# Skylarking/MARL

Hardware: AMD Instinct MI355X
Metric: env_steps_per_sec (higher is better)
Workload: dtype f32 (bf16x6 split products, fp32 accumulate)

## Files before the change

### marl_amd/csrc/qmix_fused.hip

```cpp
#include "x6.h"
#include "../../include/marl_hip.h"

namespace {

constexpr int E = 32;
constexpr int KCQ = 8;
constexpr int SS = 128 + 4;
constexpr int NAG = 5;
constexpr int PP = 136;

struct QmixArgs {
  const float *W[4], *Bv[4];
  const float *wb2, *bb2;
  ConcatSrc s;
  const float* q;
  const float* g;
  float* q_tot;
  float* dq;
  float* ws;
  const float *lr, *lterm, *lpadded, *lq_tgt;
  float gamma;
  long rows;
  int N, S, C;
};

__host__ __device__ inline long qmix_slab_floats(int C, int S) { return (long)C * (S + 1) + (E + 1) + 2; }

template <int CTRL>
__device__ __forceinline__ float dpp(float v) {
  return __builtin_bit_cast(float, __builtin_amdgcn_update_dpp(0, __builtin_bit_cast(int, v), CTRL, 0xf, 0xf, true));
}
constexpr int DPP_XOR1 = 0xB1, DPP_XOR2 = 0x4E;
constexpr int DPP_HALF_MIRROR = 0x141, DPP_MIRROR = 0x140;
constexpr int DPP_ROR4 = 0x124, DPP_ROR8 = 0x128;
template <int EW>
__device__ __forceinline__ float group_sum(float v) {
  if (EW == 4) v += dpp<DPP_ROR4>(v);
  v += dpp<DPP_ROR8>(v);
  return v;
}
template <int EW>
__device__ __forceinline__ float e_sum(float v) {
  v += dpp<DPP_XOR1>(v);
  v += dpp<DPP_XOR2>(v);
  if (EW == 8) v += dpp<DPP_HALF_MIRROR>(v);
  return v;
}
__device__ __forceinline__ float row_sum(float v) {
  v += dpp<DPP_XOR1>(v);
  v += dpp<DPP_XOR2>(v);
  v += dpp<DPP_HALF_MIRROR>(v);
  v += dpp<DPP_MIRROR>(v);
  return v;
}
__device__ __forceinline__ float sign_clamp(float x, float lo) { return __builtin_amdgcn_fmed3f(x * 0x1p126f, lo, 1.0f); }

template <bool BWD, int NW, bool LOSS = false, bool X6 = false>
__global__ __launch_bounds__(64 * NW, 2) void qmix_fused_kernel(QmixArgs a) {
  static_assert(!LOSS || BWD, "the loss is folded into the backward kernel");
  static_assert(!X6 || NW == 8, "the split variant runs eight waves (two column tiles per wave: 96 registers of pre-split weights)");
  constexpr int QNT = 64 * NW, EW = 32 / NW, GPT = 16 / EW, TPW = 8 / GPT, LT = TPW - 1;
  constexpr int SRAW = X6 ? 2 * 3 * 16 * PP * 2 : 2 * 16 * SS * 4;
  __shared__ __attribute__((aligned(16))) char Sraw[SRAW];
  float (*Ss)[16 * SS] = reinterpret_cast<float (*)[16 * SS]>(Sraw);
  short* const Sp = reinterpret_cast<short*>(Sraw);
  constexpr int PLN = 16 * PP, PBUF = 3 * PLN;
  constexpr int KR = (X6 && BWD) ? (LOSS ? 2 : 3) : 4;
  constexpr int KL = 4 - KR;
  __shared__ __attribute__((aligned(16))) i32x4 WL[KL ? NW * TPW * KL * 3 * 64 : 1];
  __shared__ __attribute__((aligned(16))) float Qt2[2][8][16];
  __shared__ __attribute__((aligned(16))) float QT[NW][16];
  __shared__ __attribute__((aligned(16))) float DQP[NW][NAG][16];
  __shared__ __attribute__((aligned(16))) float Gs2[2][16];
  __shared__ __attribute__((aligned(16))) float Ls2[2][4][16];
  const int tid = threadIdx.x, lane = tid & 63, wave = tid >> 6;
  const int q4 = lane >> 4, m = lane & 15;
  const int el = m & (EW - 1), gl = m / EW, e = EW * wave + el;
  const int N = a.N, S = a.S, C = a.C, NE = N * E;
  const bool ones = S < 128;

  f32x4 wq[X6 ? 1 : TPW][X6 ? 1 : KCQ];
  F3 wq6[X6 ? TPW : 1][X6 ? KR : 1];
  float bias[TPW];
  int grp[TPW];
#pragma unroll
  for (int c = 0; c < TPW; ++c) {
    const int g = GPT * c + gl;
    grp[c] = g;
    const float *Wp = nullptr, *Bp = nullptr;
    if (g < NAG) { if (g < N) { Wp = a.W[0] + (long)(g * E + e) * S; Bp = a.Bv[0] + g * E + e; } }
    else { Wp = a.W[g - NAG + 1] + (long)e * S; Bp = a.Bv[g - NAG + 1] + e; }
    bias[c] = Bp ? *Bp : 0.f;
    if (X6) {
#pragma unroll
      for (int kc = 0; kc < 4; ++kc) {
        float v[8];
#pragma unroll
        for (int jj = 0; jj < 8; ++jj) {
          const int kk = 32 * kc + 8 * q4 + jj;
          v[jj] = (Wp && kk < S) ? Wp[kk] : 0.f;
        }
        const F3 f = split8((f32x4){v[0], v[1], v[2], v[3]}, (f32x4){v[4], v[5], v[6], v[7]});
        if (kc < KR) wq6[c][kc < KR ? kc : 0] = f;
        else { i32x4* wl = WL + (((wave * TPW + c) * (KL ? KL : 1) + (kc - KR)) * 3) * 64 + lane; wl[0] = f.h; wl[64] = f.m; wl[128] = f.l; }
      }
    } else {
#pragma unroll
      for (int kc = 0; kc < KCQ; ++kc)
#pragma unroll
        for (int i = 0; i < 4; ++i) {
          const int kk = 16 * kc + 4 * q4 + i;
          wq[c][kc][i] = (Wp && kk < S) ? Wp[kk] : 0.f;
        }
    }
  }
  const bool is6 = grp[LT] == 6, is7 = grp[LT] == 7;
  const float wb2e = a.wb2[e];
  const float cw = is7 ? wb2e : 0.f;
  const float bb2 = a.bb2[0];
  constexpr int MT = NAG / GPT;
  const unsigned absmask = grp[MT] < NAG ? 0x7fffffffu : 0xffffffffu;
  float lo_c[TPW];
#pragma unroll
  for (int c = 0; c < TPW; ++c) lo_c[c] = grp[c] == NAG ? 1.f : (grp[c] == 7 ? 0.f : -1.f);

  f32x4 accW[BWD ? TPW : 1][BWD ? KCQ : 1];
  float sbW[TPW];
#pragma unroll
  for (int c = 0; c < TPW; ++c) sbW[c] = 0.f;
  float acc_wb2 = 0.f, acc_bb2 = 0.f;
  float acc_ln = 0.f, acc_lm = 0.f;
  if (BWD) {
#pragma unroll
    for (int c = 0; c < TPW; ++c)
#pragma unroll
      for (int kc = 0; kc < KCQ; ++kc) accW[c][kc] = (f32x4){0.f, 0.f, 0.f, 0.f};
  }
  if (tid < 2 * 8 * 16) {
    const int r8 = (tid >> 4) & 7;
    (&Qt2[0][0][0])[tid] = r8 == NAG ? 1.f : 0.f;
  }

  const int tiles = (int)((a.rows + 15) / 16);
  constexpr int NPF = 512 / QNT;
  f32x4 pf[NPF];
  int pe0 = 0, pe1 = 0, pw0 = 0, pw1 = 0;
  const int fr = tid >> 5, fc4 = (tid & 31) * 4;
  const bool ones_lane = BWD && ones && fc4 == (S & ~3);
  const int ones_j = S & 3;
  const int nrows = (int)a.rows;
  const unsigned last_row = (unsigned)(nrows - 1);
  const unsigned rpe = (unsigned)a.s.rpe0;
  const int roff = rpe ? (int)a.s.off0 : 0;
  const FastDiv fd = a.s.fd0;
  const int* emap = a.s.emap0;
  const float* sp0 = a.s.p0 + (fc4 < S ? fc4 : 0);
  const long ld = a.s.ld0, blk = (long)a.s.bs0 * a.s.ld0;
  auto map_one = [&](int tile, int i, int& pe, int& pw) {
    unsigned row = (unsigned)tile * 16u + (unsigned)(fr + (QNT / 32) * i);
    row = row < last_row ? row : last_row;
    const unsigned ep = rpe ? fastdiv(row, fd) : 0u;
    pw = (int)(row - ep * rpe) + roff;
    pe = (int)ep;
    if (emap) pe = emap[ep];
  };
  auto map_issue = [&](int tile) {
    map_one(tile, 0, pe0, pw0);
    if (NPF > 1) map_one(tile, 1, pe1, pw1);
  };
  auto fetch_one = [&](int pe, int pw) {
    f32x4 v = *reinterpret_cast<const f32x4*>(sp0 + ((long)pe * blk + (long)pw * ld));
    if (BWD) {
#pragma unroll
      for (int j = 0; j < 4; ++j) v[j] = (ones_lane && j == ones_j) ? 1.f : v[j];
    }
    return v;
  };
  auto fetch = [&](int) {
    pf[0] = fetch_one(pe0, pw0);
    if (NPF > 1) pf[NPF - 1] = fetch_one(pe1, pw1);
  };
  auto stash = [&](int buf) {
#pragma unroll
    for (int i = 0; i < NPF; ++i) {
      if (X6) {
        const F3h f = split4(pf[i]);
        short* p = Sp + buf * PBUF + (fr + (QNT / 32) * i) * PP + fc4;
        *reinterpret_cast<i32x2*>(p) = f.h;
        *reinterpret_cast<i32x2*>(p + PLN) = f.m;
        *reinterpret_cast<i32x2*>(p + 2 * PLN) = f.l;
      } else *reinterpret_cast<f32x4*>(&Ss[buf][(fr + (QNT / 32) * i) * SS + fc4]) = pf[i];
    }
  };
  float pq = 0.f, pg = 0.f, pl[4] = {0.f, 0.f, 0.f, 0.f};
  const int qr = tid / N, qn = tid - qr * N;
  auto fetch_qg = [&](int tile) {
    pq = 0.f; pg = 0.f;
    if (tid < 16 * N) {
      const int row = tile * 16 + qr;
      if (row < nrows) pq = a.q[(unsigned)(row * N + qn)];
    }
    if (BWD && tid >= 192 && tid < 208) {
      const int row = tile * 16 + (tid - 192);
      if (LOSS) {
        pl[0] = pl[1] = pl[3] = 0.f; pl[2] = 1.f;
        if (row < nrows) { pl[0] = a.lr[row]; pl[1] = a.lterm[row]; pl[2] = a.lpadded[row]; pl[3] = a.lq_tgt[row]; }
      } else if (row < nrows) pg = a.g[row];
    }
  };
  auto flush_dq = [&](int prow0) {
    if (tid < 16 * N) {
      float v = 0.f;
#pragma unroll
      for (int w = 0; w < NW; ++w) v += DQP[w][qn][qr];
      if (prow0 + qr < nrows) a.dq[(unsigned)((prow0 + qr) * N + qn)] = v;
    }
  };
  int tile = blockIdx.x;
  if (tile < tiles) {
    map_issue(tile); fetch(tile); fetch_qg(tile);
    if (tile + (int)gridDim.x < tiles) map_issue(tile + gridDim.x);
    stash(0);
  }
  int buf = 0;
  int prow0 = -1;
  ST_DECL(8);
  __syncthreads();
  for (; tile < tiles; tile += gridDim.x, buf ^= 1) {
    const int row0 = tile * 16;
    if (tid < 16 * N) Qt2[buf][qn][qr] = pq;
    if (BWD && tid >= 192 && tid < 208) {
      if (LOSS) {
#pragma unroll
        for (int k = 0; k < 4; ++k) Ls2[buf][k][tid - 192] = pl[k];
      } else Gs2[buf][tid - 192] = pg;
    }
    const int nt = tile + gridDim.x;
    if (nt < tiles) {
      fetch(nt); fetch_qg(nt);
      if (nt + (int)gridDim.x < tiles) map_issue(nt + gridDim.x);
    }
    ST_MARK(0);
    WG_BARRIER();
    ST_MARK(1);
    if (BWD && prow0 >= 0) flush_dq(prow0);
    f32x4 acc[TPW];
#pragma unroll
    for (int c = 0; c < TPW; ++c) acc[c] = (f32x4){bias[c], bias[c], bias[c], bias[c]};
    if (X6) {
      f32x4 accb[TPW];
#pragma unroll
      for (int c = 0; c < TPW; ++c) accb[c] = (f32x4){0.f, 0.f, 0.f, 0.f};
      const short* sp = Sp + buf * PBUF + m * PP + 8 * q4;
#pragma unroll
      for (int kc = 0; kc < 4; ++kc) {
        F3 xa;
        xa.h = *reinterpret_cast<const i32x4*>(sp + 32 * kc);
        xa.m = *reinterpret_cast<const i32x4*>(sp + PLN + 32 * kc);
        xa.l = *reinterpret_cast<const i32x4*>(sp + 2 * PLN + 32 * kc);
        F3 wk[TPW];
#pragma unroll
        for (int c = 0; c < TPW; ++c) {
          if (kc < KR) wk[c] = wq6[c][kc < KR ? kc : 0];
          else { const i32x4* wl = WL + (((wave * TPW + c) * (KL ? KL : 1) + (kc - KR)) * 3) * 64 + lane; wk[c].h = wl[0]; wk[c].m = wl[64]; wk[c].l = wl[128]; }
        }
#define OP(p_, q_) _Pragma("unroll") for (int c = 0; c < TPW; ++c) { if (kc & 1) accb[c] = mm(xa.p_, wk[c].q_, accb[c]); else acc[c] = mm(xa.p_, wk[c].q_, acc[c]); }
        OP(m, m) OP(h, l) OP(l, h) OP(h, m) OP(m, h) OP(h, h)
#undef OP
      }
#pragma unroll
      for (int c = 0; c < TPW; ++c) acc[c] += accb[c];
    } else {
      const float* sr = &Ss[buf][m * SS + 4 * q4];
#pragma unroll
      for (int kc = 0; kc < KCQ; ++kc) {
        const f32x4 a4 = *reinterpret_cast<const f32x4*>(sr + 16 * kc);
#pragma unroll
        for (int i = 0; i < 4; ++i)
#pragma unroll
          for (int c = 0; c < TPW; ++c) acc[c] = mfma16(a4[i], wq[c][kc][i], acc[c]);
      }
    }
    ST_MARK(2);
    __builtin_amdgcn_sched_barrier(0);
    f32x4 qv[TPW];
    f32x4 p = {0.f, 0.f, 0.f, 0.f};
#pragma unroll
    for (int c = 0; c <= MT; ++c) {
      qv[c] = *reinterpret_cast<const f32x4*>(&Qt2[buf][grp[c]][4 * q4]);
#pragma unroll
      for (int i = 0; i < 4; ++i) {
        const float av = acc[c][i];
        const float x = c < MT ? fabsf(av) : __builtin_bit_cast(float, __builtin_bit_cast(unsigned, av) & absmask);
        p[i] = c == 0 ? x * qv[c][i] : fmaf(x, qv[c][i], p[i]);
      }
    }
    f32x4 ex, hid, t4;
#pragma unroll
    for (int i = 0; i < 4; ++i) {
      p[i] = group_sum<EW>(p[i]);
      ex[i] = __expf(p[i]);
      hid[i] = p[i] > 0.f ? p[i] : ex[i] - 1.f;
      const float z = is6 ? fabsf(acc[LT][i]) : fmaxf(acc[LT][i], 0.f);
      t4[i] = row_sum(z * (is6 ? hid[i] : cw));
    }
    if (m == 0) *reinterpret_cast<f32x4*>(&QT[wave][4 * q4]) = t4;
    ST_MARK(3);
    WG_BARRIER();
    ST_MARK(4);
    if (!BWD) {
      if (tid < 16) {
        float tot = 0.f;
#pragma unroll
        for (int w = 0; w < NW; ++w) tot += QT[w][tid];
        if (row0 + tid < nrows) a.q_tot[row0 + tid] = tot + bb2;
      }
      ST_MARK(5);
    } else {
      f32x4 qt = *reinterpret_cast<const f32x4*>(&QT[0][4 * q4]);
#pragma unroll
      for (int w = 1; w < NW; ++w) qt += *reinterpret_cast<const f32x4*>(&QT[w][4 * q4]);
      f32x4 gr;
      if (LOSS) {
        const f32x4 lr = *reinterpret_cast<const f32x4*>(&Ls2[buf][0][4 * q4]);
        const f32x4 lt = *reinterpret_cast<const f32x4*>(&Ls2[buf][1][4 * q4]);
        const f32x4 lp = *reinterpret_cast<const f32x4*>(&Ls2[buf][2][4 * q4]);
        const f32x4 lq = *reinterpret_cast<const f32x4*>(&Ls2[buf][3][4 * q4]);
#pragma unroll
        for (int i = 0; i < 4; ++i) {
          qt[i] += bb2;
          const float mask = 1.f - lp[i];
          const float target = lr[i] + a.gamma * lq[i] * (1.f - lt[i]);
          const float mtd = mask * (target - qt[i]);
          gr[i] = -2.f * mask * mtd;
          acc_ln += mtd * mtd; acc_lm += mask;
        }
        if (a.q_tot && wave == 0 && m == 0) {
          if (row0 + 16 <= nrows) *reinterpret_cast<f32x4*>(&a.q_tot[row0 + 4 * q4]) = qt;
          else {
#pragma unroll
            for (int i = 0; i < 4; ++i) if (row0 + 4 * q4 + i < nrows) a.q_tot[row0 + 4 * q4 + i] = qt[i];
          }
        }
      } else gr = *reinterpret_cast<const f32x4*>(&Gs2[buf][4 * q4]);
      f32x4 dpre, dhy[TPW];
#pragma unroll
      for (int i = 0; i < 4; ++i) {
        const float w2 = group_sum<EW>(is6 ? fabsf(acc[LT][i]) : 0.f);
        dpre[i] = gr[i] * w2 * (p[i] > 0.f ? 1.f : ex[i]);
        acc_wb2 += gr[i] * fmaxf(acc[LT][i], 0.f);
        acc_bb2 += gr[i];
      }
#pragma unroll
      for (int c = 0; c < TPW; ++c) {
        const bool lo_all = GPT * c + GPT - 1 <= NAG, hi_all = GPT * c > NAG;
#pragma unroll
        for (int i = 0; i < 4; ++i) {
          float x, y;
          if (lo_all) { x = qv[c][i]; y = dpre[i]; }
          else if (hi_all) { x = gr[i]; y = is6 ? hid[i] : wb2e; }
          else {
            const bool lo = grp[c] <= NAG;
            x = lo ? qv[c][i] : gr[i];
            y = lo ? dpre[i] : (is6 ? hid[i] : wb2e);
          }
          dhy[c][i] = (x * y) * sign_clamp(acc[c][i], lo_c[c]);
        }
        if (!ones) sbW[c] += dhy[c][0] + dhy[c][1] + dhy[c][2] + dhy[c][3];
        if (GPT * c < NAG) {
          f32x4 d4;
#pragma unroll
          for (int i = 0; i < 4; ++i) d4[i] = e_sum<EW>(fabsf(acc[c][i]) * dpre[i]);
          if (el == 0 && grp[c] < N) *reinterpret_cast<f32x4*>(&DQP[wave][grp[c]][4 * q4]) = d4;
        }
      }
      ST_MARK(5);
      __builtin_amdgcn_sched_barrier(0);
      if (X6) {
        typedef __attribute__((address_space(3))) s16x4 lds_s16x4;
        F3h dA[TPW];
#pragma unroll
        for (int c = 0; c < TPW; ++c) dA[c] = split4(dhy[c]);
        const short* tb = Sp + buf * PBUF + (4 * q4 + (m >> 2)) * PP + 4 * (m & 3);
#pragma unroll
        for (int kc = 0; kc < KCQ; ++kc) {
          F3h sb;
          sb.h = __builtin_bit_cast(i32x2, __builtin_amdgcn_ds_read_tr16_b64_v4i16((lds_s16x4*)(tb + 16 * kc)));
          sb.m = __builtin_bit_cast(i32x2, __builtin_amdgcn_ds_read_tr16_b64_v4i16((lds_s16x4*)(tb + PLN + 16 * kc)));
          sb.l = __builtin_bit_cast(i32x2, __builtin_amdgcn_ds_read_tr16_b64_v4i16((lds_s16x4*)(tb + 2 * PLN + 16 * kc)));
#define OP(p_, q_) _Pragma("unroll") for (int c = 0; c < TPW; ++c) accW[c][kc] = mmh(dA[c].p_, sb.q_, accW[c][kc]);
          OP(m, m) OP(h, l) OP(l, h) OP(h, m) OP(m, h) OP(h, h)
#undef OP
        }
      } else {
        const float* sd = &Ss[buf][(4 * q4) * SS + m];
#pragma unroll
        for (int kc = 0; kc < KCQ; ++kc) {
          f32x4 sD;
#pragma unroll
          for (int i = 0; i < 4; ++i) sD[i] = sd[i * SS + 16 * kc];
#pragma unroll
          for (int i = 0; i < 4; ++i)
#pragma unroll
            for (int c = 0; c < TPW; ++c) accW[c][kc] = mfma16(dhy[c][i], sD[i], accW[c][kc]);
        }
      }
      prow0 = row0;
    }
    ST_MARK(6);
    if (nt < tiles) stash(buf ^ 1);
    ST_MARK(7);
  }
  ST_DUMP_AT(8, BWD ? 8 : 0);
  if (BWD) {
    __syncthreads();
    if (prow0 >= 0) flush_dq(prow0);
    float* slab = a.ws + (long)blockIdx.x * qmix_slab_floats(C, S);
    const int Sx = S + 1;
#pragma unroll
    for (int c = 0; c < TPW; ++c) {
#pragma unroll
      for (int i = 0; i < 4; ++i) {
        const int cc = 4 * q4 + i, g = GPT * c + cc / EW, ee = EW * wave + (cc & (EW - 1));
        if (g < NAG && g >= N) continue;
        const int col = g < NAG ? g * E + ee : NE + (g - NAG) * E + ee;
#pragma unroll
        for (int kc = 0; kc < KCQ; ++kc) {
          const int k = 16 * kc + m;
          if (k < S || (ones && k == S)) slab[(long)col * Sx + k] = accW[c][kc][i];
        }
      }
      if (!ones) {
        float sb = sbW[c];
        sb += __shfl_xor(sb, 16, 64); sb += __shfl_xor(sb, 32, 64);
        const int g = grp[c];
        if (q4 == 0 && !(g < NAG && g >= N)) slab[(long)(g < NAG ? g * E + e : NE + (g - NAG) * E + e) * Sx + S] = sb;
      }
    }
    float v = acc_wb2;
    v += __shfl_xor(v, 16, 64); v += __shfl_xor(v, 32, 64);
    if (is7 && q4 == 0) slab[(long)C * Sx + e] = v;
    float b = acc_bb2, ln = acc_ln, lm = acc_lm;
    b += __shfl_xor(b, 16, 64); b += __shfl_xor(b, 32, 64);
    ln += __shfl_xor(ln, 16, 64); ln += __shfl_xor(ln, 32, 64);
    lm += __shfl_xor(lm, 16, 64); lm += __shfl_xor(lm, 32, 64);
    if (tid == 0) {
      slab[(long)C * Sx + E] = b;
      slab[(long)C * Sx + E + 1] = LOSS ? ln : 0.f;
      slab[(long)C * Sx + E + 2] = LOSS ? lm : 0.f;
    }
  }
}

struct QmixRedArgs {
  const float* ws; int nwg; int N, S, C;
  float *dW[4], *dB[4], *dwb2, *dbb2;
  float* loss2;
};

constexpr int RSG = 16;

__global__ __launch_bounds__(64 * RSG) void qmix_fused_reduce_kernel(QmixRedArgs a) {
  __shared__ float part[RSG][64];
  const long slab = qmix_slab_floats(a.C, a.S);
  const int el = threadIdx.x & 63, sg = threadIdx.x >> 6;
  const long e = (long)blockIdx.x * 64 + el;
  float s = 0.f;
  if (e < slab) s = slab_sum(a.ws + e, slab, sg, RSG, a.nwg);
  part[sg][el] = s;
  __syncthreads();
  if (sg != 0 || e >= slab) return;
  s = 0.f;
#pragma unroll
  for (int g = 0; g < RSG; ++g) s += part[g][el];
  const int Sx = a.S + 1, NE = a.N * E;
  if (e < (long)a.C * Sx) {
    const int col = (int)(e / Sx), k = (int)(e - (long)col * Sx);
    int seg, sc;
    if (col < NE) { seg = 0; sc = col; }
    else if (col < NE + E) { seg = 1; sc = col - NE; }
    else if (col < NE + 2 * E) { seg = 2; sc = col - NE - E; }
    else { seg = 3; sc = col - NE - 2 * E; }
    if (k < a.S) a.dW[seg][(long)sc * a.S + k] += s;
    else a.dB[seg][sc] += s;
  } else {
    const long tpos = e - (long)a.C * Sx;
    if (tpos < E) a.dwb2[tpos] += s;
    else if (tpos == E) a.dbb2[0] += s;
    else if (a.loss2) a.loss2[tpos - E - 1] += s;
  }
}

}
ST_DEFINE_SETTER(marl_debug_stamps_qmix)
namespace {

inline bool supported(int N, int S, int Eq) { return Eq == E && N >= 1 && N <= NAG && S <= 128 && S >= 1; }

inline ConcatSrc state_src(const marl_src_t* s) {
  ConcatSrc c;
  c.p0 = s->p0; c.ld0 = s->ld0; c.k0 = s->k0; c.p1 = nullptr; c.ld1 = 0; c.k1 = 0;
  c.idx = nullptr; c.nhot = 0; c.hot_w = 0; c.nid = 0; c.m0 = nullptr; c.ldm0 = 0;
  c.rpe0 = s->rpe0; c.bs0 = s->bs0; c.off0 = s->off0; c.rpei = 0; c.bsi = 0; c.offi = 0;
  c.fd0 = make_fastdiv((unsigned)(s->rpe0 > 0 ? s->rpe0 : 1));
  c.fdi = make_fastdiv(1); c.fdn = make_fastdiv(1);
  c.emap0 = s->emap0;
  return c;
}

inline int fill(QmixArgs& a, const marl_qmix_weights_t* w, const marl_src_t* s, const float* q, long rows, int N, int S) {
  a.W[0] = w->w1; a.Bv[0] = w->w1_b; a.W[1] = w->b1; a.Bv[1] = w->b1_b; a.W[2] = w->w2; a.Bv[2] = w->w2_b;
  a.W[3] = w->h; a.Bv[3] = w->h_b; a.wb2 = w->b2_w; a.bb2 = w->b2_b;
  a.s = state_src(s);
  if (a.s.k0 != S || s->k1 || s->nhot || s->nid || s->m0 || (a.s.ld0 % 4) || ((uintptr_t)a.s.p0 & 15)) return 1;
  a.q = q; a.rows = rows; a.N = N; a.S = S; a.C = N * E + 3 * E;
  return 0;
}

inline unsigned grid_for(long rows, int per_cu = 1) {
  long tiles = (rows + 15) / 16;
  return (unsigned)(tiles < 256 * per_cu ? tiles : 256 * per_cu);
}

}

extern "C" int marl_qmix_fused_supported(int N, int S, int Eq) { return supported(N, S, Eq) ? 1 : 0; }

extern "C" size_t marl_qmix_fused_workspace(long rows, int N, int S) {
  return (size_t)grid_for(rows) * qmix_slab_floats(N * E + 3 * E, S) * sizeof(float);
}

static int qmix_fwd_impl(const marl_qmix_weights_t* w, const marl_src_t* s, const float* q, float* q_tot,
                         long rows, int N, int S, int Eq, bool x6, void* stream) {
  if (rows <= 0) return 0;
  if (!supported(N, S, Eq)) return (int)hipErrorInvalidValue;
  QmixArgs a;
  if (fill(a, w, s, q, rows, N, S)) return (int)hipErrorInvalidValue;
  a.g = nullptr; a.q_tot = q_tot; a.dq = nullptr; a.ws = nullptr;
  a.lr = a.lterm = a.lpadded = a.lq_tgt = nullptr; a.gamma = 0.f;
  if (x6) hipLaunchKernelGGL((qmix_fused_kernel<false, 8, false, true>), dim3(grid_for(rows, 1)), dim3(512), 0, (hipStream_t)stream, a);
  else hipLaunchKernelGGL((qmix_fused_kernel<false, 4>), dim3(grid_for(rows, 2)), dim3(256), 0, (hipStream_t)stream, a);
  MARL_CHECK_LAUNCH();
  return 0;
}
extern "C" int marl_qmix_fused_fwd(const marl_qmix_weights_t* w, const marl_src_t* s, const float* q, float* q_tot,
                                   long rows, int N, int S, int Eq, void* stream) {
  return qmix_fwd_impl(w, s, q, q_tot, rows, N, S, Eq, false, stream);
}
extern "C" int marl_qmix_fused_fwd_x6(const marl_qmix_weights_t* w, const marl_src_t* s, const float* q, float* q_tot,
                                      long rows, int N, int S, int Eq, void* stream) {
  return qmix_fwd_impl(w, s, q, q_tot, rows, N, S, Eq, true, stream);
}

static int qmix_bwd_launch(QmixArgs& a, const marl_qmix_weights_t* grads, float* loss2, float* ws, long rows, int N, int S,
                           bool loss, bool x6, hipStream_t st) {
  const unsigned nwg = grid_for(rows);
  if (x6) {
    if (loss) hipLaunchKernelGGL((qmix_fused_kernel<true, 8, true, true>), dim3(nwg), dim3(512), 0, st, a);
    else hipLaunchKernelGGL((qmix_fused_kernel<true, 8, false, true>), dim3(nwg), dim3(512), 0, st, a);
  } else if (loss) hipLaunchKernelGGL((qmix_fused_kernel<true, 8, true>), dim3(nwg), dim3(512), 0, st, a);
  else hipLaunchKernelGGL((qmix_fused_kernel<true, 8, false>), dim3(nwg), dim3(512), 0, st, a);
  MARL_CHECK_LAUNCH();
  QmixRedArgs r;
  r.ws = ws; r.nwg = (int)nwg; r.N = N; r.S = S; r.C = a.C; r.loss2 = loss2;
  r.dW[0] = const_cast<float*>(grads->w1); r.dB[0] = const_cast<float*>(grads->w1_b);
  r.dW[1] = const_cast<float*>(grads->b1); r.dB[1] = const_cast<float*>(grads->b1_b);
  r.dW[2] = const_cast<float*>(grads->w2); r.dB[2] = const_cast<float*>(grads->w2_b);
  r.dW[3] = const_cast<float*>(grads->h); r.dB[3] = const_cast<float*>(grads->h_b);
  r.dwb2 = const_cast<float*>(grads->b2_w); r.dbb2 = const_cast<float*>(grads->b2_b);
  const long slab = qmix_slab_floats(a.C, S);
  hipLaunchKernelGGL(qmix_fused_reduce_kernel, dim3((unsigned)((slab + 63) / 64)), dim3(64 * RSG), 0, st, r);
  MARL_CHECK_LAUNCH();
  return 0;
}

static int qmix_bwd_impl(const marl_qmix_weights_t* w, const marl_src_t* s, const float* q, const float* dq_tot, float* dq,
                         const marl_qmix_weights_t* grads, float* ws, size_t ws_bytes, long rows, int N, int S, int Eq, bool x6,
                         void* stream) {
  if (rows <= 0) return 0;
  if (!supported(N, S, Eq)) return (int)hipErrorInvalidValue;
  if (ws_bytes < marl_qmix_fused_workspace(rows, N, S)) return (int)hipErrorInvalidValue;
  QmixArgs a;
  if (fill(a, w, s, q, rows, N, S)) return (int)hipErrorInvalidValue;
  a.g = dq_tot; a.q_tot = nullptr; a.dq = dq; a.ws = ws;
  a.lr = a.lterm = a.lpadded = a.lq_tgt = nullptr; a.gamma = 0.f;
  return qmix_bwd_launch(a, grads, nullptr, ws, rows, N, S, false, x6, (hipStream_t)stream);
}
extern "C" int marl_qmix_fused_bwd(const marl_qmix_weights_t* w, const marl_src_t* s, const float* q,
                                   const float* dq_tot, float* dq, const marl_qmix_weights_t* grads, float* ws,
                                   size_t ws_bytes, long rows, int N, int S, int Eq, void* stream) {
  return qmix_bwd_impl(w, s, q, dq_tot, dq, grads, ws, ws_bytes, rows, N, S, Eq, false, stream);
}
extern "C" int marl_qmix_fused_bwd_x6(const marl_qmix_weights_t* w, const marl_src_t* s, const float* q,
                                      const float* dq_tot, float* dq, const marl_qmix_weights_t* grads, float* ws,
                                      size_t ws_bytes, long rows, int N, int S, int Eq, void* stream) {
  return qmix_bwd_impl(w, s, q, dq_tot, dq, grads, ws, ws_bytes, rows, N, S, Eq, true, stream);
}

static int qmix_loss_bwd_impl(const marl_qmix_weights_t* w, const marl_src_t* s, const float* q,
                              const float* q_tot_tgt, const float* r, const float* term, const float* padded,
                              float gamma, float* q_tot, float* dq, const marl_qmix_weights_t* grads,
                              float* loss2, float* ws, size_t ws_bytes, long rows, int N, int S, int Eq, bool x6,
                              void* stream) {
  if (rows <= 0) return 0;
  if (!supported(N, S, Eq) || !q_tot_tgt || !r || !term || !padded || !loss2) return (int)hipErrorInvalidValue;
  if (reinterpret_cast<uintptr_t>(q_tot) & 15) return (int)hipErrorInvalidValue;
  if (ws_bytes < marl_qmix_fused_workspace(rows, N, S)) return (int)hipErrorInvalidValue;
  QmixArgs a;
  if (fill(a, w, s, q, rows, N, S)) return (int)hipErrorInvalidValue;
  a.g = nullptr; a.q_tot = q_tot; a.dq = dq; a.ws = ws;
  a.lr = r; a.lterm = term; a.lpadded = padded; a.lq_tgt = q_tot_tgt; a.gamma = gamma;
  return qmix_bwd_launch(a, grads, loss2, ws, rows, N, S, true, x6, (hipStream_t)stream);
}
extern "C" int marl_qmix_fused_loss_bwd(const marl_qmix_weights_t* w, const marl_src_t* s, const float* q,
                                        const float* q_tot_tgt, const float* r, const float* term, const float* padded,
                                        float gamma, float* q_tot, float* dq, const marl_qmix_weights_t* grads,
                                        float* loss2, float* ws, size_t ws_bytes, long rows, int N, int S, int Eq,
                                        void* stream) {
  return qmix_loss_bwd_impl(w, s, q, q_tot_tgt, r, term, padded, gamma, q_tot, dq, grads, loss2, ws, ws_bytes, rows, N, S, Eq, false, stream);
}
extern "C" int marl_qmix_fused_loss_bwd_x6(const marl_qmix_weights_t* w, const marl_src_t* s, const float* q,
                                           const float* q_tot_tgt, const float* r, const float* term, const float* padded,
                                           float gamma, float* q_tot, float* dq, const marl_qmix_weights_t* grads,
                                           float* loss2, float* ws, size_t ws_bytes, long rows, int N, int S, int Eq,
                                           void* stream) {
  return qmix_loss_bwd_impl(w, s, q, q_tot_tgt, r, term, padded, gamma, q_tot, dq, grads, loss2, ws, ws_bytes, rows, N, S, Eq, true, stream);
}
```

Measured before the change: 66.50 million.

## Process two row tiles per iteration in the split-precision QMIX kernel

Adds a paired-tile mode for the X6 (bf16x6) path. Each loop iteration now stages, computes the hypernetwork products for, and back-propagates two 16-row tiles. Split weights held in registers or LDS are reused across both tiles, and the number of workgroup barriers per row is halved. To free registers, the backward path keeps fewer pre-split weight chunks in registers, loads biases from LDS, recomputes hid, and re-derives lane indices to lower register pressure. The prefetch and the second tile's elementwise backward are scheduled to overlap with the weight-gradient MFMAs. In exchange it uses more LDS, adds code complexity, and may increase register spills.

```diff
diff --git a/marl_amd/csrc/qmix_fused.hip b/marl_amd/csrc/qmix_fused.hip
--- a/marl_amd/csrc/qmix_fused.hip
+++ b/marl_amd/csrc/qmix_fused.hip
@@ -1,5 +1,18 @@
 #include "x6.h"
 #include "../../include/marl_hip.h"
+
+#ifndef QMIX_PAIR
+#define QMIX_PAIR 3
+#endif
+#ifndef QMIX_PAIR_PF
+#define QMIX_PAIR_PF 1
+#endif
+#ifndef QMIX_PAIR_REINDEX
+#define QMIX_PAIR_REINDEX 1
+#endif
+#ifndef QMIX_PAIR_LATE_B
+#define QMIX_PAIR_LATE_B 1
+#endif
 
 namespace {
 
@@ -55,27 +68,37 @@
 }
 __device__ __forceinline__ float sign_clamp(float x, float lo) { return __builtin_amdgcn_fmed3f(x * 0x1p126f, lo, 1.0f); }
 
+template <int V> struct IC { static constexpr int v = V; };
+template <int TPW>
+struct QTile { f32x4 acc[TPW], qv[TPW], p, ex, hid; };
+
 template <bool BWD, int NW, bool LOSS = false, bool X6 = false>
 __global__ __launch_bounds__(64 * NW, 2) void qmix_fused_kernel(QmixArgs a) {
   static_assert(!LOSS || BWD, "the loss is folded into the backward kernel");
   static_assert(!X6 || NW == 8, "the split variant runs eight waves (two column tiles per wave: 96 registers of pre-split weights)");
   constexpr int QNT = 64 * NW, EW = 32 / NW, GPT = 16 / EW, TPW = 8 / GPT, LT = TPW - 1;
-  constexpr int SRAW = X6 ? 2 * 3 * 16 * PP * 2 : 2 * 16 * SS * 4;
+  constexpr bool PAIR = X6 && ((QMIX_PAIR >> (BWD ? (LOSS ? 2 : 1) : 0)) & 1);
+  constexpr int NSL = PAIR ? 4 : 2, NQT = PAIR ? 2 : 1;
+  constexpr bool EARLY_PUT = PAIR && BWD;
+  constexpr int SRAW = X6 ? NSL * 3 * 16 * PP * 2 : 2 * 16 * SS * 4;
   __shared__ __attribute__((aligned(16))) char Sraw[SRAW];
   float (*Ss)[16 * SS] = reinterpret_cast<float (*)[16 * SS]>(Sraw);
   short* const Sp = reinterpret_cast<short*>(Sraw);
   constexpr int PLN = 16 * PP, PBUF = 3 * PLN;
-  constexpr int KR = (X6 && BWD) ? (LOSS ? 2 : 3) : 4;
+  constexpr int KR = (X6 && BWD) ? ((LOSS || PAIR) ? 2 : 3) : 4;
   constexpr int KL = 4 - KR;
   __shared__ __attribute__((aligned(16))) i32x4 WL[KL ? NW * TPW * KL * 3 * 64 : 1];
-  __shared__ __attribute__((aligned(16))) float Qt2[2][8][16];
-  __shared__ __attribute__((aligned(16))) float QT[NW][16];
-  __shared__ __attribute__((aligned(16))) float DQP[NW][NAG][16];
-  __shared__ __attribute__((aligned(16))) float Gs2[2][16];
-  __shared__ __attribute__((aligned(16))) float Ls2[2][4][16];
-  const int tid = threadIdx.x, lane = tid & 63, wave = tid >> 6;
-  const int q4 = lane >> 4, m = lane & 15;
-  const int el = m & (EW - 1), gl = m / EW, e = EW * wave + el;
+  __shared__ __attribute__((aligned(16))) float Qt2[NSL][8][16];
+  __shared__ __attribute__((aligned(16))) float QT[NQT][NW][16];
+  __shared__ __attribute__((aligned(16))) float DQP[NQT][NW][NAG][16];
+  __shared__ __attribute__((aligned(16))) float Gs2[NSL][16];
+  __shared__ __attribute__((aligned(16))) float Ls2[NSL][4][16];
+  __shared__ float Bs[EARLY_PUT ? NW * TPW * 16 : 1];
+  const int tid = threadIdx.x;
+  int lane = tid & 63, wave = tid >> 6;
+  int q4 = lane >> 4, m = lane & 15;
+  int el = m & (EW - 1);
+  const int gl = m / EW, e = EW * wave + el;
   const int N = a.N, S = a.S, C = a.C, NE = N * E;
   const bool ones = S < 128;
 
@@ -91,6 +114,7 @@
     if (g < NAG) { if (g < N) { Wp = a.W[0] + (long)(g * E + e) * S; Bp = a.Bv[0] + g * E + e; } }
     else { Wp = a.W[g - NAG + 1] + (long)e * S; Bp = a.Bv[g - NAG + 1] + e; }
     bias[c] = Bp ? *Bp : 0.f;
+    if (EARLY_PUT && q4 == 0) Bs[(wave * TPW + c) * 16 + m] = bias[c];
     if (X6) {
 #pragma unroll
       for (int kc = 0; kc < 4; ++kc) {
@@ -122,7 +146,7 @@
   const unsigned absmask = grp[MT] < NAG ? 0x7fffffffu : 0xffffffffu;
   float lo_c[TPW];
 #pragma unroll
-  for (int c = 0; c < TPW; ++c) lo_c[c] = grp[c] == NAG ? 1.f : (grp[c] == 7 ? 0.f : -1.f);
+  for (int c = 0; c < TPW; ++c) lo_c[c] = GPT * c + GPT - 1 < NAG ? -1.f : (grp[c] == NAG ? 1.f : (grp[c] == 7 ? 0.f : -1.f));
 
   f32x4 accW[BWD ? TPW : 1][BWD ? KCQ : 1];
   float sbW[TPW];
@@ -136,17 +160,18 @@
 #pragma unroll
       for (int kc = 0; kc < KCQ; ++kc) accW[c][kc] = (f32x4){0.f, 0.f, 0.f, 0.f};
   }
-  if (tid < 2 * 8 * 16) {
+  if (tid < NSL * 8 * 16) {
     const int r8 = (tid >> 4) & 7;
-    (&Qt2[0][0][0])[tid] = r8 == NAG ? 1.f : 0.f;
+    if (!EARLY_PUT || r8 >= N) (&Qt2[0][0][0])[tid] = r8 == NAG ? 1.f : 0.f;
   }
 
   const int tiles = (int)((a.rows + 15) / 16);
   constexpr int NPF = 512 / QNT;
-  f32x4 pf[NPF];
+  static_assert(!PAIR || NPF == 1, "a pair's second tile uses the second prefetch set");
+  f32x4 pf[PAIR ? 2 : NPF];
   int pe0 = 0, pe1 = 0, pw0 = 0, pw1 = 0;
-  const int fr = tid >> 5, fc4 = (tid & 31) * 4;
-  const bool ones_lane = BWD && ones && fc4 == (S & ~3);
+  int fr = tid >> 5, fc4 = (tid & 31) * 4;
+  bool ones_lane = BWD && ones && fc4 == (S & ~3);
   const int ones_j = S & 3;
   const int nrows = (int)a.rows;
   const unsigned last_row = (unsigned)(nrows - 1);
@@ -180,97 +205,154 @@
     pf[0] = fetch_one(pe0, pw0);
     if (NPF > 1) pf[NPF - 1] = fetch_one(pe1, pw1);
   };
+  auto stash_one = [&](int buf, int i, const f32x4& v) {
+    if (X6) {
+      const F3h f = split4(v);
+      short* p = Sp + buf * PBUF + (fr + (QNT / 32) * i) * PP + fc4;
+      *reinterpret_cast<i32x2*>(p) = f.h;
+      *reinterpret_cast<i32x2*>(p + PLN) = f.m;
+      *reinterpret_cast<i32x2*>(p + 2 * PLN) = f.l;
+    } else *reinterpret_cast<f32x4*>(&Ss[buf][(fr + (QNT / 32) * i) * SS + fc4]) = v;
+  };
   auto stash = [&](int buf) {
 #pragma unroll
-    for (int i = 0; i < NPF; ++i) {
-      if (X6) {
-        const F3h f = split4(pf[i]);
-        short* p = Sp + buf * PBUF + (fr + (QNT / 32) * i) * PP + fc4;
-        *reinterpret_cast<i32x2*>(p) = f.h;
-        *reinterpret_cast<i32x2*>(p + PLN) = f.m;
-        *reinterpret_cast<i32x2*>(p + 2 * PLN) = f.l;
-      } else *reinterpret_cast<f32x4*>(&Ss[buf][(fr + (QNT / 32) * i) * SS + fc4]) = pf[i];
-    }
+    for (int i = 0; i < NPF; ++i) stash_one(buf, i, pf[i]);
+  };
+  auto map_pair = [&](int tA, int tB, bool hasB) {
+    map_one(tA, 0, pe0, pw0);
+    if (hasB) map_one(tB, 0, pe1, pw1);
+  };
+  auto fetch_pair = [&](bool hasB) {
+    pf[0] = fetch_one(pe0, pw0);
+    if (hasB) pf[PAIR ? 1 : 0] = fetch_one(pe1, pw1);
+  };
+  auto stash_pair = [&](int buf, bool hasB) {
+    stash_one(buf, 0, pf[0]);
+    if (hasB) stash_one(buf + 1, 0, pf[PAIR ? 1 : 0]);
   };
   float pq = 0.f, pg = 0.f, pl[4] = {0.f, 0.f, 0.f, 0.f};
-  const int qr = tid / N, qn = tid - qr * N;
-  auto fetch_qg = [&](int tile) {
+  int tq = PAIR ? (tid & 255) : tid, qsl = PAIR ? (tid >> 8) : 0;
+  int tg = tid - 192, gsl = PAIR ? ((tg >> 4) & 1) : 0, grw = tg & 15;
+  int qr = tq / N, qn = tq - qr * N;
+  const int qpk = qn * 16 + qr;
+  auto fetch_qg = [&](int tile, int tileB = 0, bool two = false) {
     pq = 0.f; pg = 0.f;
-    if (tid < 16 * N) {
-      const int row = tile * 16 + qr;
+    if (tq < 16 * N && (two || qsl == 0)) {
+      const int row = (qsl ? tileB : tile) * 16 + qr;
       if (row < nrows) pq = a.q[(unsigned)(row * N + qn)];
     }
-    if (BWD && tid >= 192 && tid < 208) {
-      const int row = tile * 16 + (tid - 192);
+    if (BWD && tg >= 0 && tg < (two ? 32 : 16)) {
+      const int row = (gsl ? tileB : tile) * 16 + grw;
       if (LOSS) {
         pl[0] = pl[1] = pl[3] = 0.f; pl[2] = 1.f;
         if (row < nrows) { pl[0] = a.lr[row]; pl[1] = a.lterm[row]; pl[2] = a.lpadded[row]; pl[3] = a.lq_tgt[row]; }
       } else if (row < nrows) pg = a.g[row];
     }
   };
-  auto flush_dq = [&](int prow0) {
-    if (tid < 16 * N) {
+  auto put_qg = [&](int buf, bool two = false) {
+    if (tq < 16 * N && (two || qsl == 0)) Qt2[buf + qsl][qn][qr] = pq;
+    if (BWD && tg >= 0 && tg < (two ? 32 : 16)) {
+      if (LOSS) {
+#pragma unroll
+        for (int k = 0; k < 4; ++k) Ls2[buf + gsl][k][grw] = pl[k];
+      } else Gs2[buf + gsl][grw] = pg;
+    }
+  };
+  int prow0 = -1, prow1 = -1;
+  auto flush_dq = [&]() {
+    const int pr = qsl ? prow1 : prow0;
+    if (tq < 16 * N && pr >= 0) {
       float v = 0.f;
 #pragma unroll
-      for (int w = 0; w < NW; ++w) v += DQP[w][qn][qr];
-      if (prow0 + qr < nrows) a.dq[(unsigned)((prow0 + qr) * N + qn)] = v;
-    }
+      for (int w = 0; w < NW; ++w) v += DQP[qsl][w][qn][qr];
+      if (pr + qr < nrows) a.dq[(unsigned)((pr + qr) * N + qn)] = v;
+    }
+  };
+  auto reindex = [&]() {
+    int t = tid;
+    asm volatile("" : "+v"(t));
+    lane = t & 63; wave = t >> 6; q4 = lane >> 4; m = lane & 15; el = m & (EW - 1);
+    fr = t >> 5; fc4 = (t & 31) * 4;
+    ones_lane = BWD && ones && fc4 == (S & ~3);
+    sp0 = a.s.p0 + (fc4 < S ? fc4 : 0);
+    tq = t & 255; qsl = t >> 8;
+    tg = t - 192; gsl = (tg >> 4) & 1; grw = tg & 15;
+    int qo = qpk;
+    asm volatile("" : "+v"(qo));
+    qr = qo & 15; qn = qo >> 4;
   };
   int tile = blockIdx.x;
-  if (tile < tiles) {
+  const int G = (int)gridDim.x;
+  if (PAIR) {
+    if (tile < tiles) {
+      const bool hasB = tile + G < tiles;
+      map_pair(tile, tile + G, hasB); fetch_pair(hasB); fetch_qg(tile, tile + G, hasB);
+      if (tile + 2 * G < tiles) map_pair(tile + 2 * G, tile + 3 * G, tile + 3 * G < tiles);
+      stash_pair(0, hasB);
+      if (EARLY_PUT) put_qg(0, hasB);
+    }
+  } else if (tile < tiles) {
     map_issue(tile); fetch(tile); fetch_qg(tile);
-    if (tile + (int)gridDim.x < tiles) map_issue(tile + gridDim.x);
+    if (tile + G < tiles) map_issue(tile + G);
     stash(0);
   }
   int buf = 0;
-  int prow0 = -1;
   ST_DECL(8);
-  __syncthreads();
-  for (; tile < tiles; tile += gridDim.x, buf ^= 1) {
-    const int row0 = tile * 16;
-    if (tid < 16 * N) Qt2[buf][qn][qr] = pq;
-    if (BWD && tid >= 192 && tid < 208) {
-      if (LOSS) {
-#pragma unroll
-        for (int k = 0; k < 4; ++k) Ls2[buf][k][tid - 192] = pl[k];
-      } else Gs2[buf][tid - 192] = pg;
-    }
-    const int nt = tile + gridDim.x;
-    if (nt < tiles) {
-      fetch(nt); fetch_qg(nt);
-      if (nt + (int)gridDim.x < tiles) map_issue(nt + gridDim.x);
-    }
-    ST_MARK(0);
-    WG_BARRIER();
-    ST_MARK(1);
-    if (BWD && prow0 >= 0) flush_dq(prow0);
-    f32x4 acc[TPW];
-#pragma unroll
-    for (int c = 0; c < TPW; ++c) acc[c] = (f32x4){bias[c], bias[c], bias[c], bias[c]};
+  auto hyper = [&](auto nt_, int buf, QTile<TPW>* T) __attribute__((always_inline)) {
+    constexpr int NT = decltype(nt_)::v;
+#pragma unroll
+    for (int t = 0; t < NT; ++t)
+#pragma unroll
+      for (int c = 0; c < TPW; ++c) {
+        const float b = EARLY_PUT ? Bs[(wave * TPW + c) * 16 + m] : bias[c];
+        T[t].acc[c] = (f32x4){b, b, b, b};
+      }
     if (X6) {
-      f32x4 accb[TPW];
-#pragma unroll
-      for (int c = 0; c < TPW; ++c) accb[c] = (f32x4){0.f, 0.f, 0.f, 0.f};
+      f32x4 accb[NT][TPW];
+#pragma unroll
+      for (int t = 0; t < NT; ++t)
+#pragma unroll
+        for (int c = 0; c < TPW; ++c) accb[t][c] = (f32x4){0.f, 0.f, 0.f, 0.f};
       const short* sp = Sp + buf * PBUF + m * PP + 8 * q4;
 #pragma unroll
       for (int kc = 0; kc < 4; ++kc) {
-        F3 xa;
-        xa.h = *reinterpret_cast<const i32x4*>(sp + 32 * kc);
-        xa.m = *reinterpret_cast<const i32x4*>(sp + PLN + 32 * kc);
-        xa.l = *reinterpret_cast<const i32x4*>(sp + 2 * PLN + 32 * kc);
+        F3 xa[NT];
+#pragma unroll
+        for (int t = 0; t < NT; ++t) {
+          xa[t].h = *reinterpret_cast<const i32x4*>(sp + t * PBUF + 32 * kc);
+          xa[t].m = *reinterpret_cast<const i32x4*>(sp + t * PBUF + PLN + 32 * kc);
+          xa[t].l = *reinterpret_cast<const i32x4*>(sp + t * PBUF + 2 * PLN + 32 * kc);
+        }
+        if (NT == 2 && BWD && kc >= KR) {
+#pragma unroll
+          for (int c = 0; c < TPW; ++c) {
+            const i32x4* wl = WL + (((wave * TPW + c) * (KL ? KL : 1) + (kc - KR)) * 3) * 64 + lane;
+            F3 w1;
+            w1.h = wl[0]; w1.m = wl[64]; w1.l = wl[128];
+#define OP(p_, q_) _Pragma("unroll") for (int t = 0; t < NT; ++t) { \
+            if (kc & 1) accb[t][c] = mm(xa[t].p_, w1.q_, accb[t][c]); else T[t].acc[c] = mm(xa[t].p_, w1.q_, T[t].acc[c]); }
+            OP(m, m) OP(h, l) OP(l, h) OP(h, m) OP(m, h) OP(h, h)
+#undef OP
+          }
+          continue;
+        }
         F3 wk[TPW];
 #pragma unroll
         for (int c = 0; c < TPW; ++c) {
           if (kc < KR) wk[c] = wq6[c][kc < KR ? kc : 0];
           else { const i32x4* wl = WL + (((wave * TPW + c) * (KL ? KL : 1) + (kc - KR)) * 3) * 64 + lane; wk[c].h = wl[0]; wk[c].m = wl[64]; wk[c].l = wl[128]; }
         }
-#define OP(p_, q_) _Pragma("unroll") for (int c = 0; c < TPW; ++c) { if (kc & 1) accb[c] = mm(xa.p_, wk[c].q_, accb[c]); else acc[c] = mm(xa.p_, wk[c].q_, acc[c]); }
+#define OP(p_, q_) _Pragma("unroll") for (int t = 0; t < NT; ++t) _Pragma("unroll") for (int c = 0; c < TPW; ++c) { \
+          if (kc & 1) accb[t][c] = mm(xa[t].p_, wk[c].q_, accb[t][c]); else T[t].acc[c] = mm(xa[t].p_, wk[c].q_, T[t].acc[c]); }
         OP(m, m) OP(h, l) OP(l, h) OP(h, m) OP(m, h) OP(h, h)
 #undef OP
       }
 #pragma unroll
-      for (int c = 0; c < TPW; ++c) acc[c] += accb[c];
+      for (int t = 0; t < NT; ++t)
+#pragma unroll
+        for (int c = 0; c < TPW; ++c) T[t].acc[c] += accb[t][c];
     } else {
+      f32x4 (&acc)[TPW] = T[0].acc;
       const float* sr = &Ss[buf][m * SS + 4 * q4];
 #pragma unroll
       for (int kc = 0; kc < KCQ; ++kc) {
@@ -281,9 +363,10 @@
           for (int c = 0; c < TPW; ++c) acc[c] = mfma16(a4[i], wq[c][kc][i], acc[c]);
       }
     }
-    ST_MARK(2);
-    __builtin_amdgcn_sched_barrier(0);
-    f32x4 qv[TPW];
+  };
+  auto epilogue = [&](QTile<TPW>& t, int buf, int qs) __attribute__((always_inline)) {
+    f32x4 (&acc)[TPW] = t.acc;
+    f32x4 (&qv)[TPW] = t.qv;
     f32x4 p = {0.f, 0.f, 0.f, 0.f};
 #pragma unroll
     for (int c = 0; c <= MT; ++c) {
@@ -304,22 +387,24 @@
       const float z = is6 ? fabsf(acc[LT][i]) : fmaxf(acc[LT][i], 0.f);
       t4[i] = row_sum(z * (is6 ? hid[i] : cw));
     }
-    if (m == 0) *reinterpret_cast<f32x4*>(&QT[wave][4 * q4]) = t4;
-    ST_MARK(3);
-    WG_BARRIER();
-    ST_MARK(4);
-    if (!BWD) {
-      if (tid < 16) {
-        float tot = 0.f;
-#pragma unroll
-        for (int w = 0; w < NW; ++w) tot += QT[w][tid];
-        if (row0 + tid < nrows) a.q_tot[row0 + tid] = tot + bb2;
-      }
-      ST_MARK(5);
-    } else {
-      f32x4 qt = *reinterpret_cast<const f32x4*>(&QT[0][4 * q4]);
-#pragma unroll
-      for (int w = 1; w < NW; ++w) qt += *reinterpret_cast<const f32x4*>(&QT[w][4 * q4]);
+    if (m == 0) *reinterpret_cast<f32x4*>(&QT[qs][wave][4 * q4]) = t4;
+    t.p = p; t.ex = ex; t.hid = hid;
+  };
+  auto bwd_elem = [&](QTile<TPW>& t, int buf, int qs, int row0, f32x4 (&dhy)[TPW]) __attribute__((always_inline)) {
+    f32x4 (&acc)[TPW] = t.acc;
+    f32x4 (&qv)[TPW] = t.qv;
+    const f32x4 p = t.p, ex = t.ex;
+    f32x4 hid = t.hid;
+    if (PAIR) {
+#pragma unroll
+      for (int c = 0; c <= MT; ++c) qv[c] = *reinterpret_cast<const f32x4*>(&Qt2[buf][grp[c]][4 * q4]);
+#pragma unroll
+      for (int i = 0; i < 4; ++i) hid[i] = p[i] > 0.f ? p[i] : ex[i] - 1.f;
+    }
+    {
+      f32x4 qt = *reinterpret_cast<const f32x4*>(&QT[qs][0][4 * q4]);
+#pragma unroll
+      for (int w = 1; w < NW; ++w) qt += *reinterpret_cast<const f32x4*>(&QT[qs][w][4 * q4]);
       f32x4 gr;
       if (LOSS) {
         const f32x4 lr = *reinterpret_cast<const f32x4*>(&Ls2[buf][0][4 * q4]);
@@ -343,12 +428,12 @@
           }
         }
       } else gr = *reinterpret_cast<const f32x4*>(&Gs2[buf][4 * q4]);
-      f32x4 dpre, dhy[TPW];
+      f32x4 dpre;
 #pragma unroll
       for (int i = 0; i < 4; ++i) {
         const float w2 = group_sum<EW>(is6 ? fabsf(acc[LT][i]) : 0.f);
         dpre[i] = gr[i] * w2 * (p[i] > 0.f ? 1.f : ex[i]);
-        acc_wb2 += gr[i] * fmaxf(acc[LT][i], 0.f);
+        acc_wb2 = __builtin_fmaf(gr[i], fmaxf(acc[LT][i], 0.f), acc_wb2);
         acc_bb2 += gr[i];
       }
 #pragma unroll
@@ -371,11 +456,13 @@
           f32x4 d4;
 #pragma unroll
           for (int i = 0; i < 4; ++i) d4[i] = e_sum<EW>(fabsf(acc[c][i]) * dpre[i]);
-          if (el == 0 && grp[c] < N) *reinterpret_cast<f32x4*>(&DQP[wave][grp[c]][4 * q4]) = d4;
-        }
-      }
-      ST_MARK(5);
-      __builtin_amdgcn_sched_barrier(0);
+          if (el == 0 && grp[c] < N) *reinterpret_cast<f32x4*>(&DQP[qs][wave][grp[c]][4 * q4]) = d4;
+        }
+      }
+    }
+  };
+  auto dw = [&](int buf, f32x4 (&dhy)[TPW]) __attribute__((always_inline)) {
+    {
       if (X6) {
         typedef __attribute__((address_space(3))) s16x4 lds_s16x4;
         F3h dA[TPW];
@@ -405,18 +492,118 @@
             for (int c = 0; c < TPW; ++c) accW[c][kc] = mfma16(dhy[c][i], sD[i], accW[c][kc]);
         }
       }
-      prow0 = row0;
+    }
+  };
+  __syncthreads();
+  if (PAIR) {
+    for (; tile + G < tiles; tile += 2 * G, buf ^= 2) {
+      const int row0 = tile * 16, row1 = (tile + G) * 16;
+      if (BWD && QMIX_PAIR_REINDEX) reindex();
+      if (!EARLY_PUT) put_qg(buf, true);
+      const int nA = tile + 2 * G, nB = tile + 3 * G;
+      const bool hasA = nA < tiles, hasB = nB < tiles;
+      auto prefetch = [&]() {
+        if (hasA) {
+          fetch_pair(hasB); fetch_qg(nA, nB, hasB);
+          if (nA + 2 * G < tiles) map_pair(nA + 2 * G, nA + 3 * G, nA + 3 * G < tiles);
+        }
+      };
+      if (!BWD) prefetch();
+      ST_MARK(0);
+      WG_BARRIER();
+      ST_MARK(1);
+      if (BWD) flush_dq();
+      QTile<TPW> T[2];
+      hyper(IC<2>(), buf, T);
+      ST_MARK(2);
+      __builtin_amdgcn_sched_barrier(0);
+      if (BWD && QMIX_PAIR_PF == 0) { prefetch(); __builtin_amdgcn_sched_barrier(0); }
+      epilogue(T[0], buf, 0);
+      epilogue(T[1], buf + 1, 1);
+      ST_MARK(3);
+      WG_BARRIER();
+      ST_MARK(4);
+      if (!BWD) {
+        if (tid < 32) {
+          const int s = tid >> 4, r = tid & 15, row = (s ? row1 : row0) + r;
+          float tot = 0.f;
+#pragma unroll
+          for (int w = 0; w < NW; ++w) tot += QT[s][w][r];
+          if (row < nrows) a.q_tot[row] = tot + bb2;
+        }
+        ST_MARK(5);
+      } else {
+        f32x4 dhyA[TPW], dhyB[TPW];
+        bwd_elem(T[0], buf, 0, row0, dhyA);
+        if (!QMIX_PAIR_LATE_B) { __builtin_amdgcn_sched_barrier(0); bwd_elem(T[1], buf + 1, 1, row1, dhyB); }
+        ST_MARK(5);
+        __builtin_amdgcn_sched_barrier(0);
+        if (QMIX_PAIR_PF == 1) { prefetch(); __builtin_amdgcn_sched_barrier(0); }
+        dw(buf, dhyA);
+        if (QMIX_PAIR_LATE_B) {
+          __builtin_amdgcn_sched_barrier(0);
+          bwd_elem(T[1], buf + 1, 1, row1, dhyB);
+          __builtin_amdgcn_sched_barrier(0);
+        }
+        dw(buf + 1, dhyB);
+        prow0 = row0; prow1 = row1;
+      }
+      ST_MARK(6);
+      if (hasA) {
+        stash_pair(buf ^ 2, hasB);
+        if (EARLY_PUT) put_qg(buf ^ 2, hasB);
+      }
+      ST_MARK(7);
+    }
+  }
+  for (; tile < tiles; tile += G, buf ^= 1) {
+    const int row0 = tile * 16;
+    if (!EARLY_PUT) put_qg(buf);
+    const int nt = tile + G;
+    if (!PAIR && nt < tiles) {
+      fetch(nt); fetch_qg(nt);
+      if (nt + G < tiles) map_issue(nt + G);
+    }
+    ST_MARK(0);
+    WG_BARRIER();
+    ST_MARK(1);
+    if (BWD) flush_dq();
+    QTile<TPW> T[2];
+    hyper(IC<1>(), buf, T);
+    ST_MARK(2);
+    __builtin_amdgcn_sched_barrier(0);
+    epilogue(T[0], buf, 0);
+    ST_MARK(3);
+    WG_BARRIER();
+    ST_MARK(4);
+    if (!BWD) {
+      if (tid < 16) {
+        float tot = 0.f;
+#pragma unroll
+        for (int w = 0; w < NW; ++w) tot += QT[0][w][tid];
+        if (row0 + tid < nrows) a.q_tot[row0 + tid] = tot + bb2;
+      }
+      ST_MARK(5);
+    } else {
+      f32x4 dhy[TPW];
+      bwd_elem(T[0], buf, 0, row0, dhy);
+      ST_MARK(5);
+      __builtin_amdgcn_sched_barrier(0);
+      dw(buf, dhy);
+      prow0 = row0; prow1 = -1;
     }
     ST_MARK(6);
-    if (nt < tiles) stash(buf ^ 1);
+    if (!PAIR && nt < tiles) stash(buf ^ 1);
     ST_MARK(7);
   }
   ST_DUMP_AT(8, BWD ? 8 : 0);
   if (BWD) {
     __syncthreads();
-    if (prow0 >= 0) flush_dq(prow0);
+    flush_dq();
     float* slab = a.ws + (long)blockIdx.x * qmix_slab_floats(C, S);
     const int Sx = S + 1;
+    if (PAIR && QMIX_PAIR_REINDEX) reindex();
+    const int glt = m / EW, et = EW * wave + el;
 #pragma unroll
     for (int c = 0; c < TPW; ++c) {
 #pragma unroll
@@ -433,13 +620,13 @@
       if (!ones) {
         float sb = sbW[c];
         sb += __shfl_xor(sb, 16, 64); sb += __shfl_xor(sb, 32, 64);
-        const int g = grp[c];
-        if (q4 == 0 && !(g < NAG && g >= N)) slab[(long)(g < NAG ? g * E + e : NE + (g - NAG) * E + e) * Sx + S] = sb;
+        const int g = GPT * c + glt;
+        if (q4 == 0 && !(g < NAG && g >= N)) slab[(long)(g < NAG ? g * E + et : NE + (g - NAG) * E + et) * Sx + S] = sb;
       }
     }
     float v = acc_wb2;
     v += __shfl_xor(v, 16, 64); v += __shfl_xor(v, 32, 64);
-    if (is7 && q4 == 0) slab[(long)C * Sx + e] = v;
+    if (GPT * LT + glt == 7 && q4 == 0) slab[(long)C * Sx + et] = v;
     float b = acc_bb2, ln = acc_ln, lm = acc_lm;
     b += __shfl_xor(b, 16, 64); b += __shfl_xor(b, 32, 64);
     ln += __shfl_xor(ln, 16, 64); ln += __shfl_xor(ln, 32, 64);
```

After: 66.19 million. No clear change (-0.5%).
